# QEC-project-2020/MCMC-QEC-toric-RL

Hardware: AMD Instinct MI355X
Metric: MCMC sweeps/sec (whole node), L=9 toric p=0.15; eq-class histogram match (higher is better)
Workload: dtype u8

## Files before the change

### include/qecmc.h

```cpp
#ifndef QECMC_H
#define QECMC_H

#include <stddef.h>
#include <stdint.h>

#ifdef __cplusplus
extern "C" {
#endif

#define QECMC_ABI_VERSION 4

typedef enum qecmc_status {
    QECMC_OK = 0,
    QECMC_ERR_INVALID = -1,
    QECMC_ERR_NO_DEVICE = -2,
    QECMC_ERR_HIP = -3,
    QECMC_ERR_UNSUPPORTED = -4
} qecmc_status;

typedef enum qecmc_code { QECMC_TORIC = 0, QECMC_XZZX = 1, QECMC_ROTATED = 2, QECMC_PLANAR = 3 } qecmc_code;
typedef enum qecmc_scan { QECMC_SCAN_RANDOM = 0, QECMC_SCAN_SWEEP = 1, QECMC_SCAN_COLOUR = 2, QECMC_SCAN_WAVE = 3 } qecmc_scan;
typedef enum qecmc_noise { QECMC_NOISE_DEPOLARIZING = 0, QECMC_NOISE_BIASED = 1, QECMC_NOISE_ALPHA = 2 } qecmc_noise;
typedef enum qecmc_conv { QECMC_CONV_NONE = 0, QECMC_CONV_ERROR_BASED = 1 } qecmc_conv;

typedef struct qecmc_params {
    uint32_t abi_size;
    int32_t  code;
    int32_t  L;
    int32_t  Nc;
    int32_t  noise;
    int32_t  scan;
    int32_t  conv_mode;
    int32_t  device;
    uint64_t iters;
    uint64_t steps;
    int32_t  tops_burn;
    int32_t  TOPS;
    int32_t  SEQ;
    int32_t  replicas;
    double   eps;
    double   p;
    double   eta;
    double   alpha;
    double   p_logical;
    uint64_t seed;
    uint32_t first_syndrome;
    uint32_t flags;
} qecmc_params;

enum qecmc_flag {
    QECMC_FLAG_NO_PRE   = 2,
    QECMC_FLAG_NO_DELUT = 4,
    QECMC_FLAG_NO_SSW   = 8
};
#define QECMC_FLAGS_QUEUE_GRID(n) ((uint32_t)(n) << 16)

typedef struct qecmc_stats {
    uint64_t proposals;
    uint64_t swap_tests;
    double   kernel_ms;
    double   total_ms;
} qecmc_stats;

int         qecmc_abi_version(void);
const char *qecmc_last_error(void);
int         qecmc_last_kernel(int64_t key_out[10]);
int         qecmc_device_count(void);


int qecmc_apply_stabilizer(int code, int L, uint64_t N, const uint8_t *in, uint8_t *out,
                           const int32_t *rows, const int32_t *cols, const int32_t *ops, int32_t *dE);
int qecmc_apply_logical(int code, int L, uint64_t N, const uint8_t *in, uint8_t *out,
                        const int32_t *ops, const int32_t *layers, const int32_t *xpos,
                        const int32_t *zpos, int32_t *dE);
int qecmc_count_errors(int code, int L, uint64_t N, const uint8_t *in, int64_t *n);
int qecmc_eq_class(int code, int L, uint64_t N, const uint8_t *in, int32_t *cls);
int qecmc_to_class(int code, int L, uint64_t N, const uint8_t *in, uint8_t *out, const int32_t *eq);
int qecmc_syndrome(int code, int L, uint64_t N, const uint8_t *in, uint8_t *defects_out);

int qecmc_generate_syndromes(int code, int L, uint64_t N, double p_x, double p_y, double p_z, int hide_class,
                             uint64_t seed, uint32_t first_syndrome, uint8_t *init_out, uint8_t *raw_out,
                             int32_t *eq_true_out);
int qecmc_generate_syndromes_dev(int code, int L, uint64_t N, double p_x, double p_y, double p_z, int hide_class,
                                 uint64_t seed, uint32_t first_syndrome, void *d_init_out, void *d_raw_out,
                                 void *d_eq_true_out, void *hip_stream);

int qecmc_chains_from_syndromes(int code, int L, uint64_t N, const uint8_t *defects, int descend, uint8_t *chains_out,
                                uint8_t *status_out, int32_t *weight_out);
typedef struct qecmc_lift qecmc_lift;
int qecmc_lift_create(int code, int L, qecmc_lift **out);
int qecmc_lift_destroy(qecmc_lift *lift);
int qecmc_chains_from_syndromes_dev(qecmc_lift *lift, const void *d_defects, uint64_t N, int descend, void *d_chains_out,
                                    void *d_status_out , void *d_weight_out , void *hip_stream);

int qecmc_corrections(int code, int L, uint64_t N, uint32_t K, const uint8_t *candidates, const int32_t *target, int place,
                      int descend, uint8_t *corrections_out, int32_t *weight_out, int32_t *source_out, uint8_t *moved_out,
                      uint8_t *status_out);
typedef struct qecmc_corrector qecmc_corrector;
int qecmc_corrector_create(int code, int L, qecmc_corrector **out);
int qecmc_corrector_destroy(qecmc_corrector *c);
int qecmc_corrections_dev(qecmc_corrector *c, const void *d_candidates, const void *d_target, uint64_t N, uint32_t K, int place,
                          int descend, void *d_corrections_out, void *d_weight_out , void *d_source_out ,
                          void *d_moved_out , void *d_status_out , void *hip_stream);

int qecmc_coset_enumerate_info(int code, int L, int32_t *rank, int32_t *ncls, int32_t *nq, int32_t *default_chunk_bits);
int qecmc_coset_enumerate(int code, int L, uint64_t N, const uint8_t *chains, int chunk_bits, uint64_t chunk_first,
// ... 117 lines not shown
```

### mcmc-qec-toric-rl_amd/csrc/kernel_choice.hpp

```cpp
#pragma once
#include <stddef.h>
#include <stdint.h>

#include "stencil_bytes.hpp"

namespace qecmc {

constexpr int kShortRows = 18;
constexpr int kSwapFast = 64;
constexpr uint32_t kMaxGenLds = 2048;
constexpr int kLutTypes = 8;
constexpr int kGenSplit = 255;

enum LadderFlag : uint32_t {
    kConv = 1u << 0, kGsplit = 1u << 1, kBiased = 1u << 2, kScan = 1u << 3, kGentop = 1u << 4, kUset = 1u << 5, kAlpha = 1u << 6,
    kPre = 1u << 7, kDelut = 1u << 8, kQueue = 1u << 9, kSsw = 1u << 10,
};

__host__ __device__ inline int ladder_group_dwords(int Nc, int W, int ncls, int gen_dwords)
{
    int d = Nc * W * 64 + 4 * Nc * 64 + ncls * 64 + Nc * 9 + Nc * kSwapFast + 16;
    d = (d + 3) & ~3;
    return d + ((gen_dwords + 3) & ~3);
}
// ... 177 lines not shown
    const uint32_t want = kUset | (s.n_gen <= kGenSplit ? kGsplit : 0u);
    return s.Nc * 64 > 512 ? ladder_key(1024, 4, s.code, want) : ladder_key(512, 8, s.code, want);
}

inline KernelKey choose_colour(const KernelShape &s)
{
    if (s.uset) return refuse("uset: not with scan = colour");
    if (s.noise < 0 || s.noise > 2 || s.resume) return refuse("scan = colour: no resumed ladders");
    if (s.noise != 0 && s.code != kCodeXzzx && s.code != kCodeRotated) return refuse("biased / alpha rule: xzzx and rotated codes only");
    if (s.stats) {
        if (s.conv) return refuse("scan = colour: swap statistics are collected in fixed-length runs only, not with the criterion");
        if (s.Nc < 2) return refuse("swap statistics need Nc >= 2");
        return colour_stats_key(s.code, s.noise);
    }
    return colour_key(s.code, s.conv, s.noise);
}

inline bool wu_supported(const KernelShape &s)
{
    if (s.noise == 2)
        return (s.code == kCodeXzzx || s.code == kCodeRotated) && s.Nc >= 2 && s.Nc <= 16 && s.W <= 8 && s.n_gen <= 1023 && s.iters >= 1 && s.iters <= 128 &&
               s.f32ok && !s.uset && !s.resume && !s.neff && wu_plan_lds_bytes(s.Nc, s.W, s.ncls, s.L, s.conv, true, s.iters) <= 160 * 1024;
    return s.noise == 0 && s.Nc >= 2 && s.top_acc && !s.lower_acc && (s.W <= 16 || (s.W <= 32 && !s.conv && s.Nc <= 8 && s.code != kCodePlanar)) &&
           s.n_gen <= 1023 && s.iters >= 1 && s.iters <= 128 && s.swap_fast_ok && !s.uset && wu_plan_lds_bytes(s.Nc, s.W, s.ncls, s.L, s.conv, false, s.iters) <= 160 * 1024;
}
inline KernelKey choose_wave(const KernelShape &s)
{
    if (!wu_supported(s)) return refuse("scan = wave: outside what it is built for");
    const int maxt = s.Nc * 64 > 512 ? 1024 : 512, it = s.iters == 10 ? 10 : 0, wv = wu_words(s.W);
    if (s.stats) {
        if (s.conv) return refuse("scan = wave: swap statistics are collected in fixed-length runs only, not with the criterion");
        if (wv > 16) return refuse("scan = wave: no swap statistics above 16 state words per rung (the 32-word kernels' staging spills)");
        return wave_stats_key(s.code, wv, s.noise == 2);
    }
    if (s.noise == 2) return wave_key(maxt, s.conv ? 6 : 8, s.code, wv, s.conv, it, true);
    return wave_key(maxt, wv <= 12 ? 8 : 6, s.code, wv, s.conv, it, false);
}

inline bool wave_cascade_eligible(const KernelShape &s)
{
    const KernelKey k = choose_wave(s);
    return s.scan == 3 && k.ok() && k.flags == 0 && !k.conv && !k.alpha && k.wv <= 16 && s.Nc * 64 <= 512 && !(s.tune & 8) &&
           4 * wu_plan_lds_bytes(s.Nc, s.W, s.ncls, s.L, false, false, s.iters) <= 160 * 1024;
}
inline bool wave_cascade_once(const KernelShape &s) { return wave_cascade_eligible(s) && s.Nc >= 5 && s.Nc <= 7; }

constexpr bool kWalkAtEightRungs = true;
inline bool wave_cascade_walk(const KernelShape &s)
{
    if (wave_cascade_once(s)) return true;
    return kWalkAtEightRungs && s.Nc == 8 && s.iters == 10 && wave_cascade_eligible(s);
}

inline KernelKey choose_shortest(const KernelShape &s)
{
    if (s.noise != 2) return refuse("shortest-chain statistics: the alpha rule only (PTEQ_alpha_with_shortest)");
    if (s.scan != 2 && s.scan != 3) return refuse("shortest-chain statistics: scan = wave or scan = colour (scan = random: the host loop of PTEQ_alpha_with_shortest)");
    if (s.resume) return refuse("shortest-chain statistics: no resumed ladders");
    if (s.uset) return refuse("shortest-chain statistics: not with the unique-chain estimators' set");
    if (s.code != kCodeXzzx && s.code != kCodeRotated) return refuse("biased / alpha rule: xzzx and rotated codes only");
    if (s.scan == 2) return colour_short_key(s.code);
    KernelShape c = s;
    c.conv = 1; c.stats = 0;
    if (!wu_supported(c) || wu_lds_bytes(s.Nc, s.W, s.ncls, s.L, true, true, true) > 160 * 1024) return refuse("scan = wave: outside what it is built for");
    return wave_short_key(s.code, wu_words(s.W), s.iters == 10 ? 10 : 0);
}

inline KernelKey choose_kernel(const KernelShape &s)
{
    if (s.stats == 2) return choose_shortest(s);
    if (s.scan == 3) return choose_wave(s);
    if (s.scan == 2) return choose_colour(s);
    if (s.queue && !ladder_takes_queue(s)) return refuse("work queue offered to a shape without queue kernels");
    if (s.uset) return choose_ladder_uset(s);
    if (s.noise) return s.scan ? refuse("the sweep is built for the depolarizing rule only") : choose_ladder_biased(s);
    if (s.scan) return choose_ladder_sweep(s);
    return s.code == kCodeToric ? choose_ladder_toric(s) : choose_ladder_surf(s);
}

}
```

### mcmc-qec-toric-rl_amd/csrc/ladder_rs.hip

```cpp
#include "kernels.hpp"
#include "plan_host.hpp"

namespace qecmc {

namespace {

const void *kernel_of(const KernelKey &k)
{
    const void *fn = nullptr;
    for (auto unit : {ladder_toric_kernel, ladder_surf_kernel, ladder_biased_kernel, ladder_sweep_kernel, ladder_uset_kernel, colour_kernel,
                      wave_toric_kernel, wave_xzzx_kernel, wave_rotated_kernel, wave_planar_kernel, wave_alpha_kernel, wave_stats_kernel,
                      wave_stats_alpha_kernel, colour_stats_kernel, wave_shortest_kernel, colour_shortest_kernel})
        fn = fn ? fn : unit(k);
    return fn;
}

thread_local KernelKey t_last_kernel = {kRefused, 0, 0, 0, 0u, 0, 0, 0, 0, 0, nullptr};
inline void note_kernel(const KernelKey &k) { t_last_kernel = k; }

hipError_t launch_fn(const void *fn, const LadderArgs &a, hipStream_t stream, unsigned grid, size_t lds)
{
    if (lds > 64 * 1024) {
        hipError_t e = hipFuncSetAttribute(fn, hipFuncAttributeMaxDynamicSharedMemorySize, (int)lds);
        if (e != hipSuccess) return e;
    }
    void *kargs[] = {const_cast<LadderArgs *>(&a)};
    const hipError_t e = hipLaunchKernel(fn, dim3(grid), dim3((unsigned)a.Nc * 64u), kargs, lds, stream);
    return e != hipSuccess ? e : hipGetLastError();
}

}

hipError_t launch_ladder_fn(const void *fn, const KernelKey &k, const LadderArgs &a, hipStream_t stream, bool persistent)
{
    unsigned grid = (unsigned)((a.N + 63) / 64);
    if ((a.queue != nullptr) != persistent) return hipErrorInvalidValue;
    if (persistent && a.grid_cap && grid > a.grid_cap) grid = a.grid_cap;
    const size_t lds = ladder_launch_lds(kernel_shape(a));
    if (lds > 160 * 1024) return hipErrorInvalidValue;
    note_kernel(k);
    return launch_fn(fn, a, stream, grid, lds);
}

hipError_t launch_ladder(const LadderArgs &a, hipStream_t stream)
{
    if (a.N == 0) return hipSuccess;
    const KernelKey k = choose_kernel(kernel_shape(a));
    const void *fn = k.ok() ? kernel_of(k) : nullptr;
    if (!fn) return hipErrorInvalidValue;
    const bool shortest = (k.family == kFamWave || k.family == kFamColour) && k.flags == kKeyShort;
    if (shortest) {
        if (!a.short_neff || !a.short_n || !a.short_uniq || !a.short_over || !a.short_set || a.short_cap == 0 || a.short_slots < 2u * a.short_cap ||
            (a.short_slots & (a.short_slots - 1u)) || a.replicas > 1 || a.resume || a.swap_acc || a.step0 || a.nsteps == 0 || (a.conv_mode != 0 && a.nlog == nullptr))
            return hipErrorInvalidValue;
    }
    if (shortest && k.family == kFamWave) {
        if (a.wu_desc == nullptr || (a.first_syndrome & 63u) || a.bias_tbl == nullptr || a.alpha_lnb == nullptr || a.write_states) return hipErrorInvalidValue;
        LadderArgs b = a;
        b.wu_chunk = 64u; b.wu_once = 0u; b.queue = nullptr; b.grid_cap = 0u;
        note_kernel(k);
        return launch_fn(fn, b, stream, (unsigned)((a.N + 63) / 64), shortest_lds_bytes(a));
    }
    if (k.family == kFamWave) {
        if (a.wu_desc == nullptr || (a.first_syndrome & 63u) || (a.noise == 2 && (a.bias_tbl == nullptr || a.alpha_lnb == nullptr))) return hipErrorInvalidValue;
        if (k.conv && (a.nlog == nullptr || a.resume || a.write_states || a.wu_chunk < 64u || (a.wu_chunk & 63u))) return hipErrorInvalidValue;
        const uint64_t per = k.conv ? a.wu_chunk : 64u;
        LadderArgs b = a;
        b.wu_once = wave_cascade_walk(kernel_shape(a)) ? 1u : 0u;
        note_kernel(k);
        return launch_fn(fn, b, stream, (unsigned)((a.N + per - 1) / per), wu_lds_bytes(a.Nc, a.W, a.ncls, a.L, k.conv, k.alpha, false, wu_frame_steps(k.wv, k.conv, k.alpha, k.it)));
    }
    if (k.family == kFamColour) {
        if (a.phase_tab == nullptr || a.n_phases == 0 || (a.conv_mode != 0 && a.nlog == nullptr)) return hipErrorInvalidValue;
        if (a.noise != 0 && (a.col_thr == nullptr || a.bias_tbl == nullptr || (a.noise == 2 && a.alpha_lnb == nullptr))) return hipErrorInvalidValue;
        const size_t lds = shortest ? shortest_lds_bytes(a) : sizeof(uint32_t) * colour_lds_dwords(a.Nc, a.W, a.ncls, a.n_phases, a.n_gen, a.L, a.nq, a.swap_fast_ok != 0, a.noise);
        if (lds > 160 * 1024) return hipErrorInvalidValue;
        note_kernel(k);
        return launch_fn(fn, a, stream, (unsigned)a.N, lds);
    }
    return launch_ladder_fn(fn, k, a, stream, k.takes_queue());
}

bool last_launched_kernel(KernelKey &out)
{
    out = t_last_kernel;
    return t_last_kernel.ok();
}

}
```

### mcmc-qec-toric-rl_amd/csrc/ladder_wu.hpp

```cpp
#pragma once
#include "ladder_kernel.hpp"
#include "shortest_book.hpp"
#include "wu_bounds.hpp"
#include "wu_frames.hpp"

namespace qecmc {

constexpr uint32_t kWuPickStream = 0x800u;
constexpr uint32_t kSubWuPick = 9u, kSubWuAcc = 10u, kSubWuRefine = 11u;

#ifndef QECMC_WU_PRIO_SHIFT
#define QECMC_WU_PRIO_SHIFT 4
#endif
constexpr int kWuPrioShift = QECMC_WU_PRIO_SHIFT;
constexpr bool wu_prio_family(int WV, bool ALPHA) { return kWuPrioShift >= 0 && !ALPHA && WV <= 16; }
__device__ __forceinline__ void wu_step_priority(uint32_t t)
{
    constexpr uint32_t SH = kWuPrioShift < 0 ? 0u : (uint32_t)kWuPrioShift;
    uint32_t k;
    asm volatile("s_and_b32 %0, %1, %2\n\t"
                 "s_cmp_lg_u32 %0, 0\n\t"
                 "s_cbranch_scc1 4f\n\t"
                 "s_bfe_u32 %0, %1, %3\n\t"
                 "s_cmp_lg_u32 %0, 0\n\t"
// ... 364 lines not shown
    const uint8_t *src = a.resume ? a.states + (lad * NC + slot) * (uint64_t)nq : a.init + (lad / a.replicas) * (uint64_t)nq;
    uint32_t cnt = 0;
    if (w1 < 0) w1 = W;
#pragma unroll 1
    for (int w = w0; w < w1; ++w) {
        uint32_t word = 0;
#pragma unroll 4
        for (int b = 0; b < 16; ++b) {
            const int cell = w * 8 + (b >> 1), q = CODE == kCodeToric ? (cell < L * L ? (b & 1) * L * L + cell : nq) : w * 16 + b;
            if (q < nq) word |= (uint32_t)(src[q] & 3u) << (2 * b);
        }
        xrow[(w - w0) * 64] = word;
        cnt += nnz2(word);
    }
#pragma unroll 1
    for (int r = w1 - w0; r < rows; ++r) xrow[r * 64] = 0u;
    if (w0 != 0) { n4 += 4u * cnt; return; }
    n4 = 4u * cnt;
    cls = (uint32_t)(CODE == kCodeToric ? toric_eq_class_b(L, src) : surf_eq_class_b(CODE, L, src));
    if (CODE == kCodeXzzx) cls = cls == 0 ? 0u : cls == 1 ? 1u : cls == 2 ? 3u : 2u;
}

__device__ __forceinline__ void wu_bound_block(const LadderArgs &a, u32x4 &v, uint32_t trow, int i0, int left)
{
    int nql = a.nq;
    asm volatile("" : "+s"(nql));
    constexpr uint32_t RB = (uint32_t)(kSwapFast * 4);
    auto near = [&](uint32_t row) { return [row](int d) { return *(wu_lds_ptr)(uintptr_t)(row + 4u * (uint32_t)d); }; };
    uint32_t g0 = 0, g1 = 0, g2 = 0, g3 = 0;
    bool ok = true, ok1 = true, ok2 = true, ok3 = true;
    if (left > 2) {
        g0 = wu_swap_first(v.x, a.swap_inv_log2[i0], nql); g1 = wu_swap_first(v.y, a.swap_inv_log2[i0 + 1], nql);
        g2 = wu_swap_first(v.z, a.swap_inv_log2[i0 + 2], nql); g3 = wu_swap_first(v.w, a.swap_inv_log2[i0 + 3], nql);
        uint32_t a0 = near(trow)((int)g0), b0 = near(trow)((int)g0 + 1), a1 = near(trow + RB)((int)g1), b1 = near(trow + RB)((int)g1 + 1);
        uint32_t a2 = near(trow + 2u * RB)((int)g2), b2 = near(trow + 2u * RB)((int)g2 + 1), a3 = near(trow + 3u * RB)((int)g3), b3 = near(trow + 3u * RB)((int)g3 + 1);
        asm volatile("" : "+v"(a0), "+v"(b0), "+v"(a1), "+v"(b1), "+v"(a2), "+v"(b2), "+v"(a3), "+v"(b3));
        ok = wu_swap_holds(v.x, a0, b0); ok1 = wu_swap_holds(v.y, a1, b1); ok2 = wu_swap_holds(v.z, a2, b2);
        ok3 = left == 3 || wu_swap_holds(v.w, a3, b3);
    } else {
        ok = wu_swap_guess(v.x, a.swap_inv_log2[i0], nql, near(trow), g0);
        if (left > 1) ok1 = wu_swap_guess(v.y, a.swap_inv_log2[i0 + 1], nql, near(trow + RB), g1);
    }
    if (__builtin_amdgcn_ballot_w64(!(ok && ok1 && ok2 && ok3)) != 0) {
        int il = i0;
        asm volatile("" : "+s"(il));
        auto far = [&](int k) { return [&a, il, nql, k](int d) { return (uint32_t)a.swap_thr[(size_t)(il + k) * (size_t)(nql + 1) + (size_t)d]; }; };
        if (!ok) g0 = wu_swap_walk(v.x, g0, nql, near(trow), far(0));
        if (!ok1) g1 = wu_swap_walk(v.y, g1, nql, near(trow + RB), far(1));
        if (!ok2) g2 = wu_swap_walk(v.z, g2, nql, near(trow + 2u * RB), far(2));
        if (!ok3) g3 = wu_swap_walk(v.w, g3, nql, near(trow + 3u * RB), far(3));
    }
    v.x = g0; v.y = g1; v.z = g2; v.w = g3;
}

template <int CODE, int WV, bool CONV, bool QUEUE, bool TOP, int IT, bool ALPHA, bool STATS = false, bool SHORT = false, bool LONG = true>
__device__ __forceinline__ void wu_run(const LadderArgs &a, typename WuVec<WV>::type &st, WuCtx &cx, const WuEnv &ev)
{
    static_assert(!QUEUE || CONV, "the work queue serves the runs that stop by the criterion");
    static_assert(!ALPHA || CODE != kCodeToric, "the alpha rule: xzzx / rotated codes");
    static_assert(!STATS || (!CONV && WV <= 16), "the statistics kernels: fixed-length runs of up to 16 state words");
    static_assert(!SHORT || (CONV && QUEUE && ALPHA && !STATS), "the shortest-chain kernels: the alpha rule's queue kernels");
    [[maybe_unused]] uint32_t swapc = 0, nsum = 0;
    const int L = a.L;
    wu_lds_ptr const lml = (wu_lds_ptr)(uintptr_t)(ev.lds0 + ev.lml_off);
    const uint32_t lds0 = ev.lds0, slot = ev.slot, grp = ev.grp;
    const int lane = ev.lane;
    constexpr bool top = TOP;
    constexpr bool LEAN = !CONV && !ALPHA && WV <= 16;
    constexpr bool FRAME = TOP && wu_frame_steps(WV, CONV, ALPHA, IT) != 0;
    constexpr uint32_t FW = (uint32_t)WV + 1u;
    const uint32_t G = a.n_gen;
    const uint32_t m55 = 0x55555555u;
    uint32_t n4 = cx.n4, cls = cx.cls, flag = cx.flag;
    [[maybe_unused]] uint32_t nef = cx.nef;
    [[maybe_unused]] float lxyf = 0.0f, lzf = 0.0f;
    if constexpr (ALPHA) { lxyf = a.bias_l2f[ev.slot][0]; lzf = a.bias_l2f[ev.slot][1]; }
    [[maybe_unused]] const uint32_t cht_base = ev.lds0 + ev.cht_off;
    uint32_t syn = a.first_syndrome + ev.lad;
    [[maybe_unused]] uint32_t t0 = 0;
    [[maybe_unused]] uint32_t tops0 = cx.tops0, samples = 0;
    const wu_const_ptr desc = (wu_const_ptr)a.wu_desc;
    const uint32_t iters = IT ? (uint32_t)IT : a.iters;
    const uint32_t nch = (iters + 9u) / 10u, nc4 = (iters + 3u) / 4u;
    const uint32_t S = 128u / iters;
    const uint32_t thr16 = (uint32_t)((a.thr_logical + 65535u) >> 16);
    const uint32_t thr_base = lds0 + ev.thr_off;
    uint32_t nbias = 0u - (thr_base + 16u);
    asm volatile("" : "+s"(nbias));
    uint32_t pk = 0;
    [[maybe_unused]] uint32_t pa0 = 0, pa1 = 0, pb0 = 0, pb1 = 0;
    [[maybe_unused]] uint32_t pf_a = 0, pf_b = 0, pf_c = 0, pf_l = 0;
    uint32_t ws = (uint32_t)(a.step0 % S);
    uint64_t wi = a.step0 / S;
    auto refresh = [&]() {
        const u32x4 b = wu_philox(wi * 64u + (uint64_t)lane, kSubWuPick, grp, kWuPickStream + slot, a.seed_lo, a.seed_hi);
        if constexpr (FRAME) {
            constexpr uint32_t FS = (uint32_t)wu_frame_steps(WV, CONV, ALPHA, IT);
            wu_lds_rw const frm = (wu_lds_rw)(uintptr_t)(lds0 + ev.frm_off);
#pragma unroll
            for (uint32_t i = 0; i < (FS * FW + 63u) / 64u; ++i) {
                const uint32_t at = i * 64u + (uint32_t)lane;
                if (at < FS * FW) frm[at] = 0u;
            }
            __builtin_amdgcn_fence(__ATOMIC_ACQ_REL, "wavefront");
            if ((uint32_t)lane < FS * (uint32_t)IT / 2u) {
                wu_lds_rw const row = frm + ((uint32_t)lane / ((uint32_t)IT / 2u)) * FW;
                auto desc_word = [&](uint32_t g, int i) { return a.wu_desc[(size_t)g * (CODE == kCodeToric ? 8u : 16u) + (uint32_t)i]; };
                auto lml_word = [&](uint32_t kind, uint32_t pos, int w) { return lml[(kind * (uint32_t)(L + 1) + pos) * (uint32_t)WV + (uint32_t)w]; };
                auto xor_word = [&](uint32_t w, uint32_t v) { __hip_atomic_fetch_xor(row + w, v, __ATOMIC_RELAXED, __HIP_MEMORY_SCOPE_WORKGROUP); };
                wu_frame_add<CODE, WV>(b.x, b.y, thr16, G, L, desc_word, lml_word, xor_word);
                wu_frame_add<CODE, WV>(b.z, b.w, thr16, G, L, desc_word, lml_word, xor_word);
            }
            __builtin_amdgcn_fence(__ATOMIC_ACQ_REL, "wavefront");
        } else {
        const uint32_t g0 = scale_u32(b.y, G), g1 = scale_u32(b.w, G);
        pk = CODE == kCodeToric ? (g0 << 5) | (g1 << 21) : (g0 << 6) | (g1 << 22);
        if (top) { pa0 = b.x; pb0 = b.y; pa1 = b.z; pb1 = b.w; }
        }
    };
    refresh();
    constexpr bool AHEAD = LEAN && !TOP && IT == 10;
    [[maybe_unused]] u32x4 abn{0, 0, 0, 0};
    if constexpr (AHEAD) abn = wu_philox(a.step0, kSubWuAcc, syn, slot, a.seed_lo, a.seed_hi);

    for (uint64_t t = 0; QUEUE || t < a.nsteps + (CONV ? 1u : 0u); ++t) {
        if constexpr (wu_prio_family(WV, ALPHA)) wu_step_priority((uint32_t)t);
        const uint64_t T = QUEUE ? (uint64_t)((uint32_t)t - t0) : a.step0 + t;
        [[maybe_unused]] uint32_t maskv = 0, cdelta = 0;
        const uint32_t pbase = ws * iters;
        [[maybe_unused]] WuAl al{0u, 0u, 0u};
        if constexpr (ALPHA && !top) al.Nb = wu_counts_packed<WV>(st, m55, a.W);
        if constexpr (FRAME) {
            const uint32_t fv = ((wu_lds_ptr)(uintptr_t)(lds0 + ev.frm_off))[ws * FW + (uint32_t)(lane < WV ? lane : WV)];
            maskv = fv;
            cdelta = (uint32_t)__builtin_amdgcn_readlane((int)fv, WV);
        } else
        for (uint32_t c = 0; c < nch; ++c) {
            [[maybe_unused]] u32x4 ab{0, 0, 0, 0};
            if constexpr (AHEAD) ab = abn;
            else if (!top) ab = wu_philox(T * nch + c, kSubWuAcc, syn, slot, a.seed_lo, a.seed_hi);
            uint32_t left = iters - c * 10u;
            if constexpr (IT == 0) asm volatile("" : "+s"(left));
#pragma unroll
            for (int f = 0; f < 10; ++f) {
                if constexpr (IT == 0) { if ((uint32_t)f >= left) continue; }
                const uint32_t P = pbase + c * 10u + (uint32_t)f;
                if constexpr (!top && IT == 10) { if (f & 1) continue; }
                const uint32_t r = (uint32_t)__builtin_amdgcn_readlane((int)pk, IT == 10 ? (int)((pbase >> 1) + ((c * 10u + (uint32_t)f) >> 1)) : (int)(P >> 1));
                const uint32_t off = (P & 1u) ? r >> 16 : r & 0xFFFFu;
                typedef const char __attribute__((address_space(4))) *wu_const_bytes;
                const wu_const_ptr e = (wu_const_ptr)((wu_const_bytes)desc + off);
                if constexpr (top) {
                    const uint32_t A = (uint32_t)__builtin_amdgcn_readlane((int)((P & 1u) ? pa1 : pa0), (int)(P >> 1));
#define QECMC_WU_LOGICAL()                                                                                                       \
                        const uint32_t B = (uint32_t)__builtin_amdgcn_readlane((int)((P & 1u) ? pb1 : pb0), (int)(P >> 1)); \
                        const int LW = (L + 1) * WV; \
                        cdelta ^= wu_logical<CODE>(A, B, L, [&](uint32_t kind, uint32_t pos) { maskv ^= lml[kind * LW + pos * WV + lane]; });
                    if constexpr (WV == 32) {
                        const bool logical = thr16 != 0 && (A >> 16) < thr16;
                        if (logical) { QECMC_WU_LOGICAL() }
                        if constexpr (CODE == kCodeToric) {
                            const wu_desc8 d = *(wu_const_desc8)e;
                            wu_xor_cell<WV>(st, d[0], d[1], d[2], logical ? 0u : d[3], logical ? 0u : d[4], logical ? 0u : d[5]);
                        } else {
                        const uint32_t d0 = e[0], d1 = e[1], d2 = e[2], d3 = e[3];
                        const uint32_t x0 = logical ? 0u : e[4], x1 = logical ? 0u : e[5], x2 = logical ? 0u : e[6], x3 = logical ? 0u : e[7];
                        wu_xor<WV>(st, d0, d1, d2, d3, x0, x1, x2, x3);
                        }
                    } else {
                        if (thr16 != 0 && (A >> 16) < thr16) {
                            QECMC_WU_LOGICAL()
                        } else if constexpr (CODE == kCodeToric) {
                            const wu_desc8 d = *(wu_const_desc8)e;
                            wu_xor_cell<WV>(st, d[0], d[1], d[2], d[3], d[4], d[5]);
                        } else {
                            const uint32_t d0 = e[0], d1 = e[1], d2 = e[2], d3 = e[3], x0 = e[4], x1 = e[5], x2 = e[6], x3 = e[7];
// ... 43 lines not shown
                        const uint32_t d0 = e[0], d1 = e[1], d2 = e[2], d3 = e[3], x0 = e[4], x1 = e[5], x2 = e[6], x3 = e[7];
                        const uint32_t am = e[11], tlo = e[12], thi = e[13], om = e[14], coff = e[15];
                        wu_propose_alpha<CODE, WV>(a, st, al, wu_field(ab, f), cht_base + coff, lxyf, lzf, d0, d1, d2, d3, x0, x1, x2, x3, tlo, thi, om, am,
                                                   T * nc4 + (j >> 2), j & 3u, syn, slot, m55);
                    } else if constexpr (CODE == kCodeToric) {
                        const wu_desc8 d = *(wu_const_desc8)e;
                        wu_propose<CODE, WV>(st, n4, wu_field(ab, f), thr_base, nbias, d[0], 0u, d[1], d[2], d[3], 0u, d[4], d[5], d[6], 0u, 0u, 0u,
                                             T * nc4 + (j >> 2), j & 3u, syn, slot, a.seed_lo, a.seed_hi);
                    } else {
                        const uint32_t d0 = e[0], d1 = e[1], d2 = e[2], d3 = e[3], x0 = e[4], x1 = e[5], x2 = e[6], x3 = e[7], tlo = e[8];
                        const uint32_t thi = e[9], om = e[10], am = e[11];
                        wu_propose<CODE, WV>(st, n4, wu_field(ab, f), thr_base, nbias, d0, d1, d2, d3, x0, x1, x2, x3, tlo, thi, om, am,
                                             T * nc4 + (j >> 2), j & 3u, syn, slot, a.seed_lo, a.seed_hi);
                    }
                }
            }
        }
        if (top) {
            cls ^= cdelta;
            n4 = 0;
            [[maybe_unused]] uint32_t tx = 0, tz = 0, txy = 0;
#define QECMC_WU_FLUSH(w)                                                                                    \
            if constexpr (w < WV) {                                                                          \
                wu_xor_s<WV, w>(st, (uint32_t)__builtin_amdgcn_readlane((int)maskv, w));                     \
                if constexpr (ALPHA) wu_count3<WV, w>(st, tx, tz, txy, m55);                                 \
                else wu_count<WV, w>(st, n4, m55);                                                           \
            }
            WU_EACH(QECMC_WU_FLUSH)
#undef QECMC_WU_FLUSH
            if constexpr (ALPHA) { n4 = tz + txy; nef = tz | (txy << 16); }
            n4 <<= 2;
        } else if constexpr (ALPHA) {
            const wu_half2 D = __builtin_bit_cast(wu_half2, al.Dh);
            const uint32_t ez = (uint32_t)((int)((al.Nb >> 10) & 1023u) + (int)(float)D.y), exy = (uint32_t)((int)(al.Nb >> 20) + (int)(float)D.x);
            n4 = (ez + exy) << 2;
            if (al.any) nef = ez | (exy << 16);
        }
        if (++ws == S) { ws = 0; ++wi; refresh(); }

        if constexpr (LEAN) {
        int NCl = a.Nc, ncl = a.ncls;
        uint32_t slotl = ev.slot, lds0l = ev.lds0, once = a.wu_once;
        asm volatile("" : "+s"(NCl), "+s"(ncl), "+s"(slotl), "+s"(lds0l), "+s"(once));
        if constexpr (STATS || LONG) once = 0;
        const int NC = NCl;
        const uint32_t slot = slotl;
        const WuLds ol = wu_lds(NC, WV, ncl, 0, false, false);
        constexpr uint32_t xstride = (uint32_t)WV * 256u;
        const uint32_t xaddr = lds0l + (uint32_t)lane * 4u;
        wu_lds_rw const recl = (wu_lds_rw)(uintptr_t)(xaddr + (uint32_t)ol.rec * 4u), swdl = recl + NC * 64;
        const uint32_t tb0 = lds0l + (uint32_t)ol.swapT * 4u;
        const int swb = NC - 1 - (int)slot;
        constexpr bool TOPDRAWS = !LONG && wu_frame_steps(WV, CONV, ALPHA, IT) != 0;
        u32x4 sb{0, 0, 0, 0};
        [[maybe_unused]] u32x4 sb1{0, 0, 0, 0};
        [[maybe_unused]] bool duty = false;
        auto bound_block = [&](int blk, u32x4 &v) { wu_bound_block(a, v, tb0 + (uint32_t)(blk * 4) * (uint32_t)(kSwapFast * 4), blk * 4, NC - 1 - blk * 4); };
        if constexpr (TOPDRAWS && TOP) {
            sb = wu_philox(T, 0u, syn, kSwapStream, a.seed_lo, a.seed_hi);
            if (NC > 5) sb1 = wu_philox(T, 1u, syn, kSwapStream, a.seed_lo, a.seed_hi);
            bound_block(0, sb);
            if (NC > 5) bound_block(1, sb1);
        } else if constexpr (!TOPDRAWS) {
            duty = swb >= 0 && swb < 4 && swb * 4 < NC - 1;
            if (duty) {
                sb = wu_philox(T, (uint32_t)swb, syn, kSwapStream, a.seed_lo, a.seed_hi);
                bound_block(swb, sb);
            }
        }
        auto put_block = [&](int blk, const u32x4 &v) {
            wu_lds_rw p = swdl + (uint32_t)(blk * 4) * 64u;
            const int left = NC - 1 - blk * 4;
            p[0] = v.x;
            if (left > 1) p[64] = v.y;
            if (left > 2) p[128] = v.z;
            if (left > 3) p[192] = v.w;
        };
        __syncthreads();
        wu_put_all<WV>(st, xaddr + slot * xstride);
        recl[slot * 64u] = pack_info(n4 >> 2, slot, cls, flag);
        if constexpr (TOPDRAWS && TOP) {
            put_block(0, sb);
            if (NC > 5) put_block(1, sb1);
        } else if constexpr (!TOPDRAWS) {
            if (duty) put_block(swb, sb);
        }
        wu_ds_wait<WV>(st);
        __syncthreads();
        if constexpr (AHEAD) {
            abn = wu_philox(T + 1u, kSubWuAcc, syn, slot, a.seed_lo, a.seed_hi);
            asm volatile("" : "+v"(abn.x), "+v"(abn.y), "+v"(abn.z), "+v"(abn.w));
        }
        uint32_t mine;
        if (once) {
            if constexpr (TOP && !LONG) {
                wu_lds_rw const pr = recl + (NC - 8) * 64;
                wu_lds_ptr const px = swdl + (NC - 8) * 64;
                uint32_t r[8], s[7];
#pragma unroll
                for (int j = 0; j < 8; ++j) r[j] = pr[64 * (7 - j)];
#pragma unroll
                for (int j = 0; j < 7; ++j) s[j] = px[64 * (6 - j)];
                asm volatile("" : "+v"(r[0]), "+v"(r[1]), "+v"(r[2]), "+v"(r[3]), "+v"(r[4]), "+v"(r[5]), "+v"(r[6]), "+v"(r[7]),
                                  "+v"(s[0]), "+v"(s[1]), "+v"(s[2]), "+v"(s[3]), "+v"(s[4]), "+v"(s[5]), "+v"(s[6]));
#pragma unroll
                for (int j = 0; j < 7; ++j) s[j] += r[j + 1] & 0xFFFFu;
                uint32_t car = r[0], nc = car & 0xFFFFu;
#pragma unroll
                for (int j = 0; j < 7; ++j) {
                    if (j < NC - 1) {
                        const uint32_t lo = r[j + 1];
                        const bool flip = nc <= s[j];
                        pr[64 * (7 - j)] = flip ? lo : car;
                        car = flip ? car : lo;
                        nc = flip ? nc : lo & 0xFFFFu;
                    }
                }
                recl[0] = car;
            }
            __syncthreads();
            mine = recl[slot * 64u];
        } else {
            wu_lds_ptr pr = recl + (NC - 2) * 64, px = swdl + (NC - 2) * 64;
            uint32_t car = pr[64];
            for (int i = NC - 2; i >= (int)slot; --i) {
                const uint32_t lo = pr[0];
                car = wu_bound_flips(car, lo, px[0]) ? car : lo;
                pr -= 64; px -= 64;
            }
            mine = car;
            if (slot != 0) {
                const uint32_t lo = pr[0];
                if (wu_bound_flips(car, lo, px[0])) {
                    mine = lo;
                    if constexpr (STATS) swapc += 1u;
                }
            }
        }
        wu_take_all<WV>(st, xaddr + ((mine >> 16) & 0xFFu) * xstride);
        n4 = (mine & 0xFFFFu) << 2; cls = (mine >> 24) & 0x3Fu; flag = mine >> 31;
        if constexpr (STATS) nsum += mine & 0xFFFFu;
        if (top) flag = 1;
        if (slot == 0) {
            tops0 += (NC == 1) | flag;
            if (a.counts != nullptr && tops0 >= a.tops_burn) {
                wu_lds_rw const hist = (wu_lds_rw)(uintptr_t)(xaddr + (uint32_t)ol.hist * 4u);
                hist[(CODE == kCodeXzzx ? (cls ^ (cls >> 1)) : cls) * 64] += 1;
                samples++;
            }
            flag = 0;
        }
        } else {
        int NCl = a.Nc, nql = a.nq, ncl = a.ncls, Ll = a.L, Wl = a.W;
        uint32_t slotl = ev.slot, lds0l = ev.lds0;
        asm volatile("" : "+s"(NCl), "+s"(nql), "+s"(ncl), "+s"(Ll), "+s"(slotl), "+s"(lds0l), "+s"(Wl));
        const int NC = NCl, nq = nql, ncls = ncl;
        const uint32_t slot = slotl;
        const WuLds ol = wu_lds(NC, Wl, ncls, Ll, CONV, ALPHA, SHORT);
        wu_lds_rw const ldsl = (wu_lds_rw)(uintptr_t)lds0l;
        wu_lds_rw const rec = ldsl + ol.rec, swd = ldsl + ol.swd, hist = ldsl + ol.hist, swapT = ldsl + ol.swapT;
        volatile __attribute__((address_space(3))) uint32_t *const stopf = ldsl + ol.stop;
        [[maybe_unused]] wu_lds_rw const bk = ldsl + ol.bk + (uint32_t)lane, mail = ldsl + ol.mail, bot = ldsl + ol.bot, bot2 = ldsl + ol.bot2;
        [[maybe_unused]] wu_lds_drw const nefd = (wu_lds_drw)(ldsl + ol.nef) + (uint32_t)lane;
        [[maybe_unused]] wu_lds_dptr const lnbd = (wu_lds_dptr)(ldsl + ol.lnb);
        [[maybe_unused]] wu_lds_rw const skey = ldsl + ol.skey + (uint32_t)lane, sst = ldsl + ol.sst + (uint32_t)lane;
        const uint32_t xaddr = lds0l + (uint32_t)lane * 4u;
        constexpr bool PAD = WV == 32 || !CONV;
        const uint32_t xstride = (uint32_t)(WV == 32 ? kWuHalf : PAD ? WV : Wl) * 256u;
        const int swb = NC - 1 - (int)slot;
        u32x4 sb{0, 0, 0, 0};
        const bool duty = swb >= 0 && swb < 4 && swb * 4 < NC - 1;
        if (duty) sb = wu_philox(T, (uint32_t)swb, syn, kSwapStream, a.seed_lo, a.seed_hi);
        __syncthreads();
        {
            const uint32_t xo = xaddr + slot * xstride;
#define QECMC_WU_PUT(w) if constexpr (w < WV && w < kWuHalf) { if (WV == 32 || !CONV || w < wu_words_min(WV) || w < Wl) wu_ds_write<WV, w>(st, xo); }
#define QECMC_WU_PUT_HI(w) if constexpr (w < WV && w >= kWuHalf) wu_ds_write<WV, w, w - kWuHalf>(st, xo);
            WU_EACH(QECMC_WU_PUT)
            rec[slot * 64u + (uint32_t)lane] = pack_info(n4 >> 2, slot, cls, flag);
            if constexpr (ALPHA) nefd[slot * 64u] = alpha_neff(nef, a.alpha);
            if (duty) {
                wu_lds_rw p = swd + (uint32_t)(swb * 4) * 64u + (uint32_t)lane;
                const int left = NC - 1 - swb * 4;
                p[0] = sb.x;
                if (left > 1) p[64] = sb.y;
                if (left > 2) p[128] = sb.z;
                if (left > 3) p[192] = sb.w;
            }
        }
        wu_ds_wait<WV>(st);
        __syncthreads();
        if constexpr (CONV) { if (stopf[t & 1]) break; }
// ... 254 lines not shown
```

### mcmc-qec-toric-rl_amd/csrc/tables_test_api.cpp

```cpp
#include "class_sweep.hpp"
#include "class_sweep_cut.hpp"
#include "class_sweep_tiled.hpp"
#include "class_sweep_site.hpp"
#include "class_minplus.hpp"
#include "class_minplus_trace.hpp"
#include "class_minplus_site.hpp"
#include "class_minplus_tiled.hpp"
#include "corrections.hpp"
#include "enumerate.hpp"
#include "kernel_choice.hpp"
#include "plan_host.hpp"
#include "syndrome_lift.hpp"
#include "tables.hpp"
#include "wu_bounds.hpp"
#include "wu_frames.hpp"

#include <cstdio>
#include <cstring>

using namespace qecmc;
using namespace qecmc::tables;

namespace {
template <class T> int put(const std::vector<T> &v, T *out, int cap)
// ... 37 lines not shown
uint64_t qt_thr44(double v) { return thr44(v); }
uint32_t qt_thr32(double v) { return thr32(v); }
double qt_chain_factor(double p) { return chain_factor(p); }
int qt_ladder(double p_bottom, double p_top, int Nc, double *pl, double *pd)
{
    std::vector<double> a, b;
    ladder_probabilities(p_bottom, p_top, Nc, a, b);
    std::memcpy(pl, a.data(), a.size() * sizeof(double));
    if (!b.empty()) std::memcpy(pd, b.data(), b.size() * sizeof(double));
    return (int)b.size();
}
int qt_bias_tables(int alpha_model, double p, double eta_or_alpha, int nq, double *out, int cap)
{
    return put(alpha_model ? alpha_tables(p, eta_or_alpha, (size_t)nq) : bias_tables(p, eta_or_alpha, (size_t)nq), out, cap);
}
int qt_patterns(int code, int L, uint8_t *gen_type, int cap_types, uint32_t *patterns, int cap_patterns)
{
    std::vector<uint8_t> gt;
    std::vector<uint32_t> pat;
    generator_patterns(gen_table(code, L), gt, pat);
    if (put(gt, gen_type, cap_types) < 0) return -1;
    return put(pat, patterns, cap_patterns);
}
int qt_count_change(const uint32_t *patterns, int n, uint32_t *out, int cap)
{
    return put(count_change_table(std::vector<uint32_t>(patterns, patterns + n)), out, cap);
}
int qt_swap_thresholds(const double *pdiff, int n, int nq, uint64_t *out, int cap)
{
    return put(swap_thresholds(std::vector<double>(pdiff, pdiff + n), nq), out, cap);
}
int qt_colour_phases(int code, int L, uint16_t *out, int cap)
{
    int n_phases = 0;
    const std::vector<uint16_t> ph = colour_phases(gen_table(code, L), n_phases);
    return put(ph, out, cap) < 0 ? -1 : n_phases;
}
void qt_choose_kernels(const KernelShape *shapes, int n, int64_t *keys)
{
    for (int i = 0; i < n; ++i) {
        const KernelKey k = choose_kernel(shapes[i]);
        const int64_t v[11] = {k.family, k.maxt, k.minw, k.code, k.flags, k.wv, k.conv, k.it, k.alpha, k.rule, (int64_t)(intptr_t)k.why};
        std::memcpy(keys + 11 * (size_t)i, v, sizeof v);
    }
}
void qt_wave_cascade_once(const KernelShape *shapes, int n, int32_t *once)
{
    for (int i = 0; i < n; ++i) once[i] = wave_cascade_once(shapes[i]) ? 1 : 0;
}
void qt_wave_cascade_walk(const KernelShape *shapes, int n, int32_t *walk)
{
    for (int i = 0; i < n; ++i) walk[i] = wave_cascade_walk(shapes[i]) ? 1 : 0;
}
int qt_kernel_shape_ints(void) { return (int)(sizeof(KernelShape) / sizeof(int)); }
int qt_plan_dims(const qecmc_params *p, int32_t *shape_ints, char *msg, int msg_cap)
{
    HostPlan hp;
    Refusal r = validate_params(p);
    if (!r.code) r = plan_dims(*p, hp);
    KernelShape s = {};
    if (!r.code) {
        s = kernel_shape(hp.args);
        s.gen_type = !hp.gen_type.empty();
    }
    return answer(r, s, shape_ints, msg, msg_cap);
}
int qt_plan(const qecmc_params *p, int cu_count, int32_t *shape_ints, uint64_t *lds_bytes, uint32_t *grid, char *msg, int msg_cap)
{
    HostPlan hp;
    Refusal r = validate_params(p);
    if (!r.code) r = plan_host(*p, hp);
    if (!r.code) { *lds_bytes = hp.lds_bytes; *grid = queue_grid(hp, cu_count, p->flags); }
    return answer(r, hp.shape, shape_ints, msg, msg_cap);
}
int qt_plan_key_equal(const qecmc_params *a, const qecmc_params *b)
{
    const qecmc_params ka = plan_key(*a), kb = plan_key(*b);
    return std::memcmp(&ka, &kb, sizeof ka) == 0;
}
int qt_plan_equal(const qecmc_params *pa, const qecmc_params *pb)
{
    HostPlan a, b;
    if (validate_params(pa).code || validate_params(pb).code || plan_host(*pa, a).code || plan_host(*pb, b).code) return -1;
    a.args.seed_lo = a.args.seed_hi = b.args.seed_lo = b.args.seed_hi = 0;
    return std::memcmp(&a.args, &b.args, sizeof a.args) == 0 && a.gen == b.gen && a.xyz_lut == b.xyz_lut && a.wu_desc == b.wu_desc && a.col_thr == b.col_thr &&
           a.lmask == b.lmask && a.acc_top == b.acc_top && a.gen_type == b.gen_type && a.phases == b.phases && a.bias == b.bias && a.lnb == b.lnb &&
           a.swap_thr == b.swap_thr && same_shape(a.shape, b.shape) && a.lds_bytes == b.lds_bytes && a.takes_queue == b.takes_queue &&
           a.queue_family == b.queue_family && a.queue_per_cu == b.queue_per_cu;
}
uint64_t qt_workspace_need(const qecmc_params *p, uint32_t grid, uint64_t N, int queue) { return workspace_need(*p, grid, N, queue != 0); }
void qt_resume_conv_bytes(const qecmc_params *p, uint64_t N, uint64_t log_rows, uint64_t *record_bytes, uint64_t *log_bytes)
{
    const ResumeConvBytes need = resume_conv_need(*p, N, log_rows);
    *record_bytes = need.record;
    *log_bytes = need.log;
}
int qt_resume_conv_check(const qecmc_params *p, char *msg, int msg_cap)
{
    const Refusal r = resume_conv_check(*p);
    if (msg && msg_cap > 0) std::snprintf(msg, (size_t)msg_cap, "%s", r.msg.c_str());
    return r.code;
}
int qt_rng_range_check(int resume, uint64_t step0, uint64_t nsteps, uint64_t prop0, uint64_t iters, char *msg, int msg_cap)
{
    const Refusal r = resume ? rng_range_check_resume("resume", step0, nsteps, iters) : rng_range_check("step", step0, nsteps, prop0, iters);
    if (msg && msg_cap > 0) std::snprintf(msg, (size_t)msg_cap, "%s", r.msg.c_str());
// ... 361 lines not shown
```

### mcmc-qec-toric-rl_amd/qecmc/_lib.py

```python
import ctypes as C
import os

import numpy as np

_HERE = os.path.dirname(os.path.abspath(__file__))
LIB_PATH = os.path.join(_HERE, "libqecmc.so")
FLAG_NO_PRE, FLAG_NO_DELUT, FLAG_NO_SSW = 2, 4, 8


def dev_flags(switches=0, queue_grid=0):
    return (int(switches) & 0xFFFF) | (int(queue_grid) << 16)


def use_library(path):
    global LIB_PATH, _lib
    if _lib is not None:
        raise QecmcError("use_library() after the library has been loaded")
    LIB_PATH = os.path.abspath(path)

TORIC, XZZX, ROTATED, PLANAR = 0, 1, 2, 3
SCAN_RANDOM, SCAN_SWEEP, SCAN_COLOUR, SCAN_WAVE = 0, 1, 2, 3
SCANS = {"random": SCAN_RANDOM, "sweep": SCAN_SWEEP, "colour": SCAN_COLOUR, "wave": SCAN_WAVE}
NOISE_DEPOLARIZING, NOISE_BIASED, NOISE_ALPHA = 0, 1, 2
CONV_NONE, CONV_ERROR_BASED = 0, 1
PTDC_INIT_PER_DROPLET, PTDC_SET_PER_RUNG = 1, 2


class QecmcError(RuntimeError):
    pass


class Params(C.Structure):
    _fields_ = [("abi_size", C.c_uint32), ("code", C.c_int32), ("L", C.c_int32), ("Nc", C.c_int32),
                ("noise", C.c_int32), ("scan", C.c_int32), ("conv_mode", C.c_int32), ("device", C.c_int32),
                ("iters", C.c_uint64), ("steps", C.c_uint64), ("tops_burn", C.c_int32), ("TOPS", C.c_int32),
                ("SEQ", C.c_int32), ("replicas", C.c_int32), ("eps", C.c_double), ("p", C.c_double),
                ("eta", C.c_double), ("alpha", C.c_double), ("p_logical", C.c_double), ("seed", C.c_uint64),
                ("first_syndrome", C.c_uint32), ("flags", C.c_uint32)]


class Stats(C.Structure):
    _fields_ = [("proposals", C.c_uint64), ("swap_tests", C.c_uint64), ("kernel_ms", C.c_double),
                ("total_ms", C.c_double)]


_u8p = C.POINTER(C.c_uint8)
_i32p = C.POINTER(C.c_int32)
_u32p = C.POINTER(C.c_uint32)
_i64p = C.POINTER(C.c_int64)
_u16p = C.POINTER(C.c_uint16)
_u64p = C.POINTER(C.c_uint64)

SIGNATURES = {
    "qecmc_abi_version": (C.c_int, []),
    "qecmc_last_error": (C.c_char_p, []),
    "qecmc_last_kernel": (C.c_int, [_i64p]),
    "qecmc_device_count": (C.c_int, []),
    "qecmc_apply_stabilizer": (C.c_int, [C.c_int, C.c_int, C.c_uint64, _u8p, _u8p, _i32p, _i32p, _i32p, _i32p]),
    "qecmc_apply_logical": (C.c_int, [C.c_int, C.c_int, C.c_uint64, _u8p, _u8p, _i32p, _i32p, _i32p, _i32p, _i32p]),
    "qecmc_count_errors": (C.c_int, [C.c_int, C.c_int, C.c_uint64, _u8p, _i64p]),
# ... 175 lines not shown
```

Before: 8.122 billion.

## Spread swap-bound computation across rungs in eight-rung wave cascade

```diff
diff --git a/include/qecmc.h b/include/qecmc.h
--- a/include/qecmc.h
+++ b/include/qecmc.h
@@ -51,7 +51,8 @@
 enum qecmc_flag {
     QECMC_FLAG_NO_PRE   = 2,
     QECMC_FLAG_NO_DELUT = 4,
-    QECMC_FLAG_NO_SSW   = 8
+    QECMC_FLAG_NO_SSW   = 8,
+    QECMC_FLAG_NO_SPREAD = 16
 };
 #define QECMC_FLAGS_QUEUE_GRID(n) ((uint32_t)(n) << 16)
 
diff --git a/mcmc-qec-toric-rl_amd/csrc/kernel_choice.hpp b/mcmc-qec-toric-rl_amd/csrc/kernel_choice.hpp
--- a/mcmc-qec-toric-rl_amd/csrc/kernel_choice.hpp
+++ b/mcmc-qec-toric-rl_amd/csrc/kernel_choice.hpp
@@ -253,6 +253,14 @@
     return kWalkAtEightRungs && s.Nc == 8 && s.iters == 10 && wave_cascade_eligible(s);
 }
 
+constexpr uint32_t kSpreadRungs = 1u << 8;
+inline int wave_cascade_mode(const KernelShape &s)
+{
+    if (!wave_cascade_walk(s)) return 0;
+    const bool topdraws = s.Nc <= 8 && wu_frame_steps(wu_words(s.W), s.conv != 0, s.noise == 2, s.iters == 10 ? 10 : 0) != 0;
+    return topdraws && ((kSpreadRungs >> s.Nc) & 1u) && !(s.tune & 16) ? 2 : 1;
+}
+
 inline KernelKey choose_shortest(const KernelShape &s)
 {
     if (s.noise != 2) return refuse("shortest-chain statistics: the alpha rule only (PTEQ_alpha_with_shortest)");
diff --git a/mcmc-qec-toric-rl_amd/csrc/ladder_rs.hip b/mcmc-qec-toric-rl_amd/csrc/ladder_rs.hip
--- a/mcmc-qec-toric-rl_amd/csrc/ladder_rs.hip
+++ b/mcmc-qec-toric-rl_amd/csrc/ladder_rs.hip
@@ -66,7 +66,7 @@
         if (k.conv && (a.nlog == nullptr || a.resume || a.write_states || a.wu_chunk < 64u || (a.wu_chunk & 63u))) return hipErrorInvalidValue;
         const uint64_t per = k.conv ? a.wu_chunk : 64u;
         LadderArgs b = a;
-        b.wu_once = wave_cascade_walk(kernel_shape(a)) ? 1u : 0u;
+        b.wu_once = (uint32_t)wave_cascade_mode(kernel_shape(a));
         note_kernel(k);
         return launch_fn(fn, b, stream, (unsigned)((a.N + per - 1) / per), wu_lds_bytes(a.Nc, a.W, a.ncls, a.L, k.conv, k.alpha, false, wu_frame_steps(k.wv, k.conv, k.alpha, k.it)));
     }
diff --git a/mcmc-qec-toric-rl_amd/csrc/ladder_wu.hpp b/mcmc-qec-toric-rl_amd/csrc/ladder_wu.hpp
--- a/mcmc-qec-toric-rl_amd/csrc/ladder_wu.hpp
+++ b/mcmc-qec-toric-rl_amd/csrc/ladder_wu.hpp
@@ -440,6 +440,31 @@
     }
     v.x = g0; v.y = g1; v.z = g2; v.w = g3;
 }
+__device__ __forceinline__ uint32_t wu_bound_word(const LadderArgs &a, uint32_t x, uint32_t trow, int i)
+{
+    int nql = a.nq;
+    asm volatile("" : "+s"(nql));
+    auto near = [trow](int d) { return *(wu_lds_ptr)(uintptr_t)(trow + 4u * (uint32_t)d); };
+    uint32_t g;
+    const bool ok = wu_swap_guess(x, a.swap_inv_log2[i], nql, near, g);
+    if (__builtin_amdgcn_ballot_w64(!ok) != 0) {
+        int il = i;
+        asm volatile("" : "+s"(il));
+        if (!ok) g = wu_swap_walk(x, g, nql, near, [&a, il, nql](int d) { return (uint32_t)a.swap_thr[(size_t)il * (size_t)(nql + 1) + (size_t)d]; });
+    }
+    return g;
+}
+__device__ __forceinline__ void wu_put_block(wu_lds_rw p, const u32x4 &v, int left)
+{
+    p[0] = v.x;
+    if (left > 1) p[64] = v.y;
+    if (left > 2) p[128] = v.z;
+    if (left > 3) p[192] = v.w;
+}
+#ifndef QECMC_WU_SPREAD_AT
+#define QECMC_WU_SPREAD_AT 0
+#endif
+constexpr int kWuSpreadAt = QECMC_WU_SPREAD_AT;
 
 template <int CODE, int WV, bool CONV, bool QUEUE, bool TOP, int IT, bool ALPHA, bool STATS = false, bool SHORT = false, bool LONG = true>
 __device__ __forceinline__ void wu_run(const LadderArgs &a, typename WuVec<WV>::type &st, WuCtx &cx, const WuEnv &ev)
@@ -510,6 +535,24 @@
     constexpr bool AHEAD = LEAN && !TOP && IT == 10;
     [[maybe_unused]] u32x4 abn{0, 0, 0, 0};
     if constexpr (AHEAD) abn = wu_philox(a.step0, kSubWuAcc, syn, slot, a.seed_lo, a.seed_hi);
+    constexpr bool SPREAD = LEAN && !STATS && !LONG && wu_frame_steps(WV, CONV, ALPHA, IT) != 0;
+    if constexpr (SPREAD) {
+        if (a.wu_once == 2u) {
+            const int NC = a.Nc;
+            const WuLds ol = wu_lds(NC, WV, a.ncls, 0, false, false);
+            const uint32_t col = lds0 + (uint32_t)lane * 4u;
+            if constexpr (TOP) {
+                wu_lds_rw const swd0 = (wu_lds_rw)(uintptr_t)(col + (uint32_t)ol.swd * 4u);
+                wu_put_block(swd0, wu_philox(a.step0, 0u, syn, kSwapStream, a.seed_lo, a.seed_hi), NC - 1);
+                if (NC > 5) wu_put_block(swd0 + 256, wu_philox(a.step0, 1u, syn, kSwapStream, a.seed_lo, a.seed_hi), NC - 5);
+            }
+            __syncthreads();
+            if constexpr (!TOP && kWuSpreadAt == 0) {
+                wu_lds_rw const row = (wu_lds_rw)(uintptr_t)(col + (uint32_t)(ol.swd + (int)slot * 64) * 4u);
+                row[0] = wu_bound_word(a, row[0], lds0 + (uint32_t)(ol.swapT + (int)slot * kSwapFast) * 4u, (int)slot);
+            }
+        }
+    }
 
     for (uint64_t t = 0; QUEUE || t < a.nsteps + (CONV ? 1u : 0u); ++t) {
         if constexpr (wu_prio_family(WV, ALPHA)) wu_step_priority((uint32_t)t);
@@ -659,15 +702,21 @@
         const uint32_t tb0 = lds0l + (uint32_t)ol.swapT * 4u;
         const int swb = NC - 1 - (int)slot;
         constexpr bool TOPDRAWS = !LONG && wu_frame_steps(WV, CONV, ALPHA, IT) != 0;
+        const bool spread = once == 2u;
         u32x4 sb{0, 0, 0, 0};
         [[maybe_unused]] u32x4 sb1{0, 0, 0, 0};
         [[maybe_unused]] bool duty = false;
         auto bound_block = [&](int blk, u32x4 &v) { wu_bound_block(a, v, tb0 + (uint32_t)(blk * 4) * (uint32_t)(kSwapFast * 4), blk * 4, NC - 1 - blk * 4); };
         if constexpr (TOPDRAWS && TOP) {
-            sb = wu_philox(T, 0u, syn, kSwapStream, a.seed_lo, a.seed_hi);
-            if (NC > 5) sb1 = wu_philox(T, 1u, syn, kSwapStream, a.seed_lo, a.seed_hi);
-            bound_block(0, sb);
-            if (NC > 5) bound_block(1, sb1);
+            if (spread) {
+                sb = wu_philox(T + 1u, 0u, syn, kSwapStream, a.seed_lo, a.seed_hi);
+                if (NC > 5) sb1 = wu_philox(T + 1u, 1u, syn, kSwapStream, a.seed_lo, a.seed_hi);
+            } else {
+                sb = wu_philox(T, 0u, syn, kSwapStream, a.seed_lo, a.seed_hi);
+                if (NC > 5) sb1 = wu_philox(T, 1u, syn, kSwapStream, a.seed_lo, a.seed_hi);
+                bound_block(0, sb);
+                if (NC > 5) bound_block(1, sb1);
+            }
         } else if constexpr (!TOPDRAWS) {
             duty = swb >= 0 && swb < 4 && swb * 4 < NC - 1;
             if (duty) {
@@ -675,20 +724,20 @@
                 bound_block(swb, sb);
             }
         }
-        auto put_block = [&](int blk, const u32x4 &v) {
-            wu_lds_rw p = swdl + (uint32_t)(blk * 4) * 64u;
-            const int left = NC - 1 - blk * 4;
-            p[0] = v.x;
-            if (left > 1) p[64] = v.y;
-            if (left > 2) p[128] = v.z;
-            if (left > 3) p[192] = v.w;
+        auto put_block = [&](int blk, const u32x4 &v) { wu_put_block(swdl + (uint32_t)(blk * 4) * 64u, v, NC - 1 - blk * 4); };
+        [[maybe_unused]] auto own_bound = [&]() {
+            wu_lds_rw const row = swdl + slot * 64u;
+            row[0] = wu_bound_word(a, row[0], tb0 + slot * (uint32_t)(kSwapFast * 4), (int)slot);
         };
+        if constexpr (TOPDRAWS && !TOP && kWuSpreadAt == 1) { if (spread) own_bound(); }
         __syncthreads();
         wu_put_all<WV>(st, xaddr + slot * xstride);
         recl[slot * 64u] = pack_info(n4 >> 2, slot, cls, flag);
         if constexpr (TOPDRAWS && TOP) {
-            put_block(0, sb);
-            if (NC > 5) put_block(1, sb1);
+            if (!spread) {
+                put_block(0, sb);
+                if (NC > 5) put_block(1, sb1);
+            }
         } else if constexpr (!TOPDRAWS) {
             if (duty) put_block(swb, sb);
         }
@@ -710,6 +759,12 @@
                 for (int j = 0; j < 7; ++j) s[j] = px[64 * (6 - j)];
                 asm volatile("" : "+v"(r[0]), "+v"(r[1]), "+v"(r[2]), "+v"(r[3]), "+v"(r[4]), "+v"(r[5]), "+v"(r[6]), "+v"(r[7]),
                                   "+v"(s[0]), "+v"(s[1]), "+v"(s[2]), "+v"(s[3]), "+v"(s[4]), "+v"(s[5]), "+v"(s[6]));
+                if constexpr (TOPDRAWS) {
+                    if (spread) {
+                        put_block(0, sb);
+                        if (NC > 5) put_block(1, sb1);
+                    }
+                }
 #pragma unroll
                 for (int j = 0; j < 7; ++j) s[j] += r[j + 1] & 0xFFFFu;
                 uint32_t car = r[0], nc = car & 0xFFFFu;
@@ -745,6 +800,7 @@
             }
         }
         wu_take_all<WV>(st, xaddr + ((mine >> 16) & 0xFFu) * xstride);
+        if constexpr (TOPDRAWS && !TOP && kWuSpreadAt == 0) { if (spread) own_bound(); }
         n4 = (mine & 0xFFFFu) << 2; cls = (mine >> 24) & 0x3Fu; flag = mine >> 31;
         if constexpr (STATS) nsum += mine & 0xFFFFu;
         if (top) flag = 1;
diff --git a/mcmc-qec-toric-rl_amd/csrc/tables_test_api.cpp b/mcmc-qec-toric-rl_amd/csrc/tables_test_api.cpp
--- a/mcmc-qec-toric-rl_amd/csrc/tables_test_api.cpp
+++ b/mcmc-qec-toric-rl_amd/csrc/tables_test_api.cpp
@@ -113,6 +113,10 @@
 {
     for (int i = 0; i < n; ++i) walk[i] = wave_cascade_walk(shapes[i]) ? 1 : 0;
 }
+void qt_wave_cascade_mode(const KernelShape *shapes, int n, int32_t *mode)
+{
+    for (int i = 0; i < n; ++i) mode[i] = wave_cascade_mode(shapes[i]);
+}
 int qt_kernel_shape_ints(void) { return (int)(sizeof(KernelShape) / sizeof(int)); }
 int qt_plan_dims(const qecmc_params *p, int32_t *shape_ints, char *msg, int msg_cap)
 {
diff --git a/mcmc-qec-toric-rl_amd/qecmc/_lib.py b/mcmc-qec-toric-rl_amd/qecmc/_lib.py
--- a/mcmc-qec-toric-rl_amd/qecmc/_lib.py
+++ b/mcmc-qec-toric-rl_amd/qecmc/_lib.py
@@ -5,7 +5,7 @@
 
 _HERE = os.path.dirname(os.path.abspath(__file__))
 LIB_PATH = os.path.join(_HERE, "libqecmc.so")
-FLAG_NO_PRE, FLAG_NO_DELUT, FLAG_NO_SSW = 2, 4, 8
+FLAG_NO_PRE, FLAG_NO_DELUT, FLAG_NO_SSW, FLAG_NO_SPREAD = 2, 4, 8, 16
 
 
 def dev_flags(switches=0, queue_grid=0):
```

Result: faster. 8.294 billion (median of 6 runs) (+2.1%).
